# sdace9719/marl-soccer

Hardware: NVIDIA B200
Metric: env_steps_per_sec (higher is better)
Workload: dtype f32

## Files before the change

marl_soccer_b200/csrc/msoc.cu:

```cuda
#include <cuda_runtime.h>
#include <cuda_bf16.h>
#include <stdint.h>
#include <stdio.h>
#include <stdlib.h>
#include <string.h>
#include <atomic>
#include <string>
#include <vector>

#include "../../include/msoc.h"
#include "step_core.cuh"
#include "render_core.cuh"

using namespace msoc;

#ifdef MSOC_CHECKS
__device__ unsigned int g_msoc_check_bits;
#endif

static thread_local std::string g_last_error;
static std::atomic<uint64_t> g_launches{0};

static int fail(int code, const char *what, cudaError_t ce = cudaSuccess)
{
    char buf[512];
    if (ce != cudaSuccess) snprintf(buf, sizeof buf, "%s: %s", what, cudaGetErrorString(ce));
    else snprintf(buf, sizeof buf, "%s", what);
    g_last_error = buf;
    return code;
}
#define CUDA_TRY(expr)                                                        \
    do {                                                                      \
        cudaError_t _e = (expr);                                              \
        if (_e != cudaSuccess) return fail(MSOC_ERR_CUDA, #expr, _e);         \
    } while (0)

struct DeviceGuard {
    int prev = -1;
    explicit DeviceGuard(int dev) { cudaGetDevice(&prev); if (prev != dev) cudaSetDevice(dev); else prev = -1; }
    ~DeviceGuard() { if (prev >= 0) cudaSetDevice(prev); }
};

constexpr int MAX_CHUNKS = 8;
enum { CTL_LIGHT = 0, CTL_HEAVY = 1, CTL_NEXT_BATCH = 2, CTL_PAIR = 4, CTL_MULTI = 5, CTL_WORDS = 8 };
enum { CTL_STEP_FAST = 16, CTL_STEP_CONTACT = 17, CTL_LAST_COUNTS = 20 , CTL_CHUNK0 = 24, CTL_TOTAL = CTL_CHUNK0 + CTL_WORDS * MAX_CHUNKS };

struct msoc_handle {
    int device;
    int64_t n;
    uint64_t global_offset;
    SimCfg cfg;
    Arrays A;
    int sm_count, blocks_per_sm;
    int blocks_per_sm_teams;
    int heavy_lanes_override;
    void *slab;
    float *d_obs, *d_act, *d_rew;
    uint8_t *d_done, *d_mask;
    int8_t *d_goal;
    int32_t *d_score;
    double *d_stats;
    int *d_ctl;
    int *d_list;
    int *d_list2;
    float *d_frames;
    void *d_inject;
    cudaStream_t pipe_stream;
    cudaEvent_t ev_pipe_fork, ev_pipe_join;
    void *d_stage; size_t stage_bytes;
};

constexpr int WARPS_PER_BLOCK = 4;
constexpr int BLOCK = WARPS_PER_BLOCK * 32;

constexpr int ENV_STRIDE = SCRATCH_WORDS | 1;
constexpr int OBS_ENVS = 8;
constexpr int BLOCK_WORDS = OBS_ENVS * 4 * OBS;
constexpr int REC_F4 = 7;
constexpr int RECS_WORDS = OBS_ENVS * 3 * REC_F4 * 4;
constexpr int STAGE_WORDS = BLOCK_WORDS + RECS_WORDS;

struct StepParams {
    Arrays A;
    SimCfg cfg;
    const float *actions;
    float *obs_out;
    float *frames_out;
    float *reward;
    uint8_t *done;
    int8_t *goal;
    int32_t *score;
    double *stats;
    int *ctl;
    int *list;
    int *list2;
    int64_t e0, e1;
    uint64_t global_offset;
    uint32_t flags;
    int heavy_lanes;
    int chunk;
};

#ifdef MSOC_TIMELINE
__device__ unsigned long long g_tl[1 << 18];
__device__ unsigned int g_tl_n;
extern "C" int msoc_debug_timeline(unsigned long long *out, unsigned int *n) {
    cudaMemcpyFromSymbol(n, g_tl_n, sizeof(unsigned int)); unsigned int z = 0; cudaMemcpyToSymbol(g_tl_n, &z, sizeof z);
    return (int)cudaMemcpyFromSymbol(out, g_tl, sizeof g_tl);
}
__device__ __forceinline__ unsigned long long gtime() { unsigned long long t; asm volatile("mov.u64 %0, %%globaltimer;" : "=l"(t)); return t; }
__device__ __forceinline__ void tl_record(int kid, unsigned long long t0) {
    const unsigned int i = atomicAdd(&g_tl_n, 1u);
    unsigned int smid; asm volatile("mov.u32 %0, %%smid;" : "=r"(smid));
    if (i < (1u << 16)) { g_tl[4 * i] = (unsigned long long)kid; g_tl[4 * i + 1] = t0; g_tl[4 * i + 2] = gtime(); g_tl[4 * i + 3] = smid; }
}
#define MSOC_TL_BEGIN() const unsigned long long tl0 = gtime()
#define MSOC_TL_END(kid) do { if (lane == 0) tl_record(kid, tl0); } while (0)
#else
#define MSOC_TL_BEGIN() do { } while (0)
#define MSOC_TL_END(kid) do { } while (0)
#endif
struct Tally { int done, goals_b, goals_r, contacts, overflow, nonfinite; float ret; };
__device__ __forceinline__ void tally_clear(Tally &T) { T.done = T.goals_b = T.goals_r = T.contacts = T.overflow = T.nonfinite = 0; T.ret = 0.0f; }

__device__ __forceinline__ int *step_ctl(const StepParams &P, int step) { return P.chunk < 0 ? P.ctl + CTL_WORDS * (step & 1) : P.ctl + CTL_CHUNK0 + CTL_WORDS * P.chunk; }

template <bool TEAMS>
__device__ __forceinline__ bool step_one_env(const int MODE, const int ALLOWED, const StepParams &P, int step, int64_t e, Work &W, int &load, Tally &T)
{
    float act[12];
    const float4 *a4 = reinterpret_cast<const float4 *>(P.actions + e * 12);
    const float4 x0 = __ldg(a4), x1 = __ldg(a4 + 1), x2 = __ldg(a4 + 2);
    act[0] = x0.x; act[1] = x0.y; act[2] = x0.z; act[3] = x0.w;
    act[4] = x1.x; act[5] = x1.y; act[6] = x1.z; act[7] = x1.w;
    act[8] = x2.x; act[9] = x2.y; act[10] = x2.z; act[11] = x2.w;
    bool finite = true;
#pragma unroll
    for (int k = 0; k < 12; k++) finite = finite && (fabsf(act[k]) <= 3.0e38f);
    Env E;
    const float4 *rec = P.A.pose[buf_cur(step)] + e * POSE_F4;
    if ((ALLOWED & (1 << MODE_FULL)) && MODE == MODE_FULL) {
        if (__float_as_uint(rec[7].z) & FLAG_INJECT) rec = P.A.inject + e * POSE_F4;
    }
    load_env(P.A, rec, e, E);
    StepOut out;
    if (!env_step<TEAMS>(MODE, ALLOWED, E, act, P.cfg, P.A, cache_half(step), e, P.global_offset + (uint64_t)e, P.flags, W, out, load)) return false;
    if (TEAMS) reinterpret_cast<float4 *>(P.reward)[e] = make_float4(out.reward, out.reward, out.reward_r, out.reward_r);
    else reinterpret_cast<float2 *>(P.reward)[e] = make_float2(out.reward, out.reward);
    P.done[e] = out.done;
    P.goal[e] = out.goal;
    if (P.score != nullptr) reinterpret_cast<int2 *>(P.score)[e] = make_int2(out.score_b, out.score_r);
    store_env(P.A, buf_next(step), e, E, out.score_dirty);
    if (out.fresh_episode) {
        store_env_record(P.A.pose[buf_cur(step)] + e * POSE_F4, E);
        store_env_record(P.A.pose[buf_prev(step)] + e * POSE_F4, E);
    }
    T.nonfinite += finite ? 0 : 1;
    T.done += out.done; T.goals_b += out.goal > 0; T.goals_r += out.goal < 0;
    T.contacts += out.n_contacts; T.overflow += out.overflow; T.ret += out.finished_return;
    return true;
}

__device__ __forceinline__ void bulk_store(void *gdst, const void *ssrc, uint32_t bytes)
{
    asm volatile("cp.async.bulk.global.shared::cta.bulk_group [%0], [%1], %2;" ::"l"(gdst), "r"((uint32_t)__cvta_generic_to_shared(ssrc)), "r"(bytes) : "memory");
}
__device__ __forceinline__ void bulk_commit() { asm volatile("cp.async.bulk.commit_group;" ::: "memory"); }
__device__ __forceinline__ void bulk_wait_read() { asm volatile("cp.async.bulk.wait_group.read 0;" ::: "memory"); }
__device__ __forceinline__ void fence_async_smem() { asm volatile("fence.proxy.async.shared::cta;" ::: "memory"); }

struct RecLoad { float4 v[6]; };
__device__ __forceinline__ void fetch_slot(int r, int lane, int &k, int &e8, int &f)
{
    const int sl = r * 32 + lane;
    k = sl / (OBS_ENVS * REC_F4);
    const int rem = sl - k * (OBS_ENVS * REC_F4);
    e8 = rem / REC_F4; f = rem - e8 * REC_F4;
}
__device__ __forceinline__ void obs_fetch(const Arrays &A, int step, uint32_t mask, int g, int my_env, int lane, RecLoad &R)
{
    const uint32_t m8 = (mask >> (8 * g)) & 0xffu;
#pragma unroll
    for (int r = 0; r < 6; r++) {
        int k, e8, f;
        fetch_slot(r, lane, k, e8, f);
        const int env = __shfl_sync(0xffffffffu, my_env, (8 * g + e8) & 31);
        R.v[r] = make_float4(0.0f, 0.0f, 0.0f, 0.0f);
        if ((r < 5 || lane < 3 * OBS_ENVS * REC_F4 - 160) && ((m8 >> e8) & 1u)) {
            const int b = k == 0 ? buf_prev(step) : k == 1 ? buf_cur(step) : buf_next(step);
            const float4 *p = A.pose[b] + (int64_t)env * POSE_F4 + f;
            R.v[r] = k == 2 ? __ldcg(p) : *p;
        }
    }
}
__device__ __forceinline__ void obs_tile(const Arrays &A, const SimCfg &cfg, float *obs_out, float *frames_out, int step, float *s_stage,
                                         uint32_t lane_mask, int64_t my_env64, int lane)
{
    const int a = lane & 3, el = lane >> 2;
    float4 *recs4 = reinterpret_cast<float4 *>(s_stage + BLOCK_WORDS);
    float2 *mine = reinterpret_cast<float2 *>(s_stage) + lane * 33;
    __syncwarp();
    uint32_t mask = lane_mask;
    int my_env = (int)my_env64;
    if (lane_mask != 0xffffffffu) {
        int *s_idx = reinterpret_cast<int *>(s_stage);
        if ((lane_mask >> lane) & 1u) s_idx[__popc(lane_mask & ((1u << lane) - 1u))] = my_env;
        __syncwarp();
// ... 8 lines not shown
#pragma unroll 1
    while (true) {
        const uint32_t m8 = (mask >> (8 * g)) & 0xffu;
#pragma unroll
        for (int r = 0; r < 6; r++)
            if (r < 5 || lane < 3 * OBS_ENVS * REC_F4 - 160) recs4[r * 32 + lane] = R.v[r];
        __syncwarp();
        int gn = g + 1;
        while (gn < 4 && ((mask >> (8 * gn)) & 0xffu) == 0u) gn++;
        if (gn < 4) obs_fetch(A, step, mask, gn, my_env, lane, R);
        const int env = __shfl_sync(0xffffffffu, my_env, 8 * g + el);
        if ((m8 >> el) & 1u) {
            MSOC_CHECK(env >= 0 && env < A.n, CHK_OBS_ENV);
#pragma unroll
            for (int k = 0; k < 3; k++) {
                float o[22];
                frame_of_record(recs4 + (k * OBS_ENVS + el) * REC_F4, a, cfg, o);
#pragma unroll
                for (int i = 0; i < 11; i++) mine[k * 11 + i] = make_float2(o[2 * i], o[2 * i + 1]);
            }
        }
        fence_async_smem();
        __syncwarp();
        if (a == 0 && ((m8 >> el) & 1u))
            bulk_store(obs_out + (int64_t)env * (4 * OBS), s_stage + el * (4 * OBS), 4 * OBS * sizeof(float));
        bulk_commit();
        if (frames_out != nullptr) {
            float2 *fr2 = reinterpret_cast<float2 *>(frames_out);
            const float2 *stage2 = reinterpret_cast<const float2 *>(s_stage);
#pragma unroll
            for (int it = 0; it < 11; it++) {
                const int idx = it * 32 + lane;
                const int row = idx / 11, j = idx - row * 11;
                const int env2 = __shfl_sync(0xffffffffu, my_env, 8 * g + (row >> 2));
                if ((m8 >> (row >> 2)) & 1u) fr2[(int64_t)env2 * 44 + (row & 3) * 11 + j] = stage2[row * 33 + 22 + j];
            }
        }
        bulk_wait_read();
        __syncwarp();
        if (gn >= 4) break;
        g = gn;
    }
}

#ifndef MSOC_FAST_BLOCK
#define MSOC_FAST_BLOCK 128
#endif
constexpr int FAST_BLOCK = MSOC_FAST_BLOCK;
constexpr size_t FAST_SMEM_BYTES = (size_t)(FAST_BLOCK / 32) * STAGE_WORDS * sizeof(float);
#ifndef MSOC_FAST_MIN_BLOCKS
#define MSOC_FAST_MIN_BLOCKS 4
#endif

__device__ __forceinline__ void flush_tally(const Tally &T, double *stats, int lane)
{
    int nd = T.done, gb = T.goals_b, gr = T.goals_r, nc = T.contacts, ov = T.overflow, nf = T.nonfinite;
    float ret = T.ret;
    if (!__any_sync(0xffffffffu, (nd | gb | gr | nc | ov | nf) != 0)) return;
#pragma unroll
    for (int o = 16; o > 0; o >>= 1) {
        nd += __shfl_xor_sync(0xffffffffu, nd, o); gb += __shfl_xor_sync(0xffffffffu, gb, o);
        gr += __shfl_xor_sync(0xffffffffu, gr, o); nc += __shfl_xor_sync(0xffffffffu, nc, o);
        ov += __shfl_xor_sync(0xffffffffu, ov, o);
        nf += __shfl_xor_sync(0xffffffffu, nf, o);
        ret += __shfl_xor_sync(0xffffffffu, ret, o);
    }
    if (lane == 0) {
        if (nd) { atomicAdd(stats + 0, (double)nd); atomicAdd(stats + 1, (double)ret); }
        if (gb) atomicAdd(stats + 2, (double)gb);
        if (gr) atomicAdd(stats + 3, (double)gr);
        if (nc) atomicAdd(stats + 5, (double)nc);
        if (ov) atomicAdd(stats + 6, (double)ov);
        if (nf) atomicAdd(stats + 7, (double)nf);
    }
}

template <bool TEAMS>
__global__ void __launch_bounds__(FAST_BLOCK, MSOC_FAST_MIN_BLOCKS) msoc_step_fast_kernel(const __grid_constant__ StepParams P)
{
    extern __shared__ __align__(16) float s_dyn[];
    const int tid = threadIdx.x, warp = tid >> 5, lane = tid & 31;
    float *s_warp = s_dyn + warp * STAGE_WORDS;
    cudaGridDependencySynchronize();
    const int step = P.ctl[CTL_STEP_FAST];
    int *ctl = step_ctl(P, step);
    if (blockIdx.x == 0) {
        if (P.chunk < 0 && tid < CTL_WORDS) P.ctl[CTL_WORDS * ((step & 1) ^ 1) + tid] = 0;
        if (tid == 0) {
            P.ctl[CTL_STEP_CONTACT] = step;
            atomicAdd(P.stats + 4, (double)(P.e1 - P.e0));
        }
    }
    MSOC_TL_BEGIN();
    const int64_t my_env = P.e0 + (int64_t)blockIdx.x * FAST_BLOCK + tid;
    const bool have = my_env < P.e1;
    Tally T; tally_clear(T);
    Work W;
    W.ovf = nullptr; W.body = W.pool = W.geom = W.old = W.isl = nullptr; W.pool_count = nullptr;
    bool ok = false;
    int load = 0;
    if (have) {
        asm volatile("prefetch.global.L2 [%0];" ::"l"(P.A.pose[buf_prev(step)] + my_env * POSE_F4));
        ok = step_one_env<TEAMS>(MODE_FAST, 1 << MODE_FAST, P, step, my_env, W, load, T);
    }
    const uint32_t mask = __ballot_sync(0xffffffffu, ok);
    const bool declined = have && !ok;
    const uint32_t mdec = __ballot_sync(0xffffffffu, declined);
    uint32_t mclass = 0u;
    int base = 0;
    if (mdec != 0u) {
        const uint32_t b0 = __ballot_sync(0xffffffffu, declined && (load & 1)), b1 = __ballot_sync(0xffffffffu, declined && (load & 2));
        auto class_mask = [&](int cl) { return mdec & ((cl & 1) ? b0 : ~b0) & ((cl & 2) ? b1 : ~b1); };
        mclass = class_mask(load);
        const uint32_t of_lane = class_mask(lane & 3);
        if (lane < N_LOADS && of_lane != 0u) {
            const int word = lane == LOAD_LIGHT ? CTL_LIGHT : lane == LOAD_HEAVY ? CTL_HEAVY : lane == LOAD_PAIR ? CTL_PAIR : CTL_MULTI;
            base = atomicAdd(ctl + word, __popc(of_lane));
        }
    }
    if (mask != 0u) obs_tile(P.A, P.cfg, P.obs_out, P.frames_out, step, s_warp, mask, my_env, lane);
    if (mdec != 0u) {
        base = __shfl_sync(0xffffffffu, base, declined ? load : 0);
        if (declined) {
            const int rank = base + __popc(mclass & ((1u << lane) - 1u));
            int *lst = (load == LOAD_LIGHT || load == LOAD_HEAVY) ? P.list : P.list2;
            const bool front = load == LOAD_LIGHT || load == LOAD_PAIR;
            lst[front ? P.e0 + rank : P.e1 - 1 - rank] = (int)my_env;
        }
    }
    flush_tally(T, P.stats, lane);
    if ((blockIdx.x & 15) == 0 && warp == 0) MSOC_TL_END(0);
}

static_assert(STAGE_WORDS <= 32 * ENV_STRIDE, "the observation staging must fit the per-warp solver scratch");
#ifndef MSOC_HEAVY_BLOCK
#define MSOC_HEAVY_BLOCK 64
#endif
constexpr int HEAVY_BLOCK = MSOC_HEAVY_BLOCK;
#ifndef MSOC_HEAVY_MIN_BLOCKS
#define MSOC_HEAVY_MIN_BLOCKS 4
#endif
constexpr int HEAVY_MIN_BLOCKS = MSOC_HEAVY_MIN_BLOCKS;

constexpr int HEAVY_WARP_WORDS = (32 * ENV_STRIDE + 3) & ~3;
constexpr size_t STEP_SMEM_BYTES = (size_t)(HEAVY_BLOCK / 32) * HEAVY_WARP_WORDS * sizeof(float);

template <int MODES, bool TEAMS>
__device__ __forceinline__ void contact_body(const StepParams &P, int *s_pool_count)
{
    extern __shared__ __align__(16) float s_dyn[];
    const int tid = threadIdx.x, warp = tid >> 5, lane = tid & 31;
    float *s_warp = s_dyn + warp * HEAVY_WARP_WORDS;
    cudaGridDependencySynchronize();
    const int step = P.ctl[CTL_STEP_CONTACT];
    int *ctl = step_ctl(P, step);
    if (P.chunk < 0 && blockIdx.x == 0 && tid == 0) {
        P.ctl[CTL_STEP_FAST] = (step + 1) % 6;
        P.ctl[CTL_LAST_COUNTS + 0] = ctl[CTL_LIGHT]; P.ctl[CTL_LAST_COUNTS + 1] = ctl[CTL_HEAVY];
        P.ctl[CTL_LAST_COUNTS + 2] = ctl[CTL_PAIR]; P.ctl[CTL_LAST_COUNTS + 3] = ctl[CTL_MULTI];
    }
    const int n_heavy = (MODES & (1 << MODE_FULL)) ? ctl[CTL_HEAVY] : 0, n_multi = (MODES & (1 << MODE_MULTI)) ? ctl[CTL_MULTI] : 0;
    const int n_pair = (MODES & (1 << MODE_PAIR)) ? ctl[CTL_PAIR] : 0, n_light = (MODES & (1 << MODE_LIGHT)) ? ctl[CTL_LIGHT] : 0;
    MSOC_CHECK(step >= 0 && step < 6, CHK_STEP_COUNTER);
    MSOC_CHECK(n_heavy >= 0 && n_light >= 0 && (int64_t)n_heavy + n_light <= P.e1 - P.e0, CHK_LIST_COUNT);
    MSOC_CHECK(n_multi >= 0 && n_pair >= 0 && (int64_t)n_multi + n_pair <= P.e1 - P.e0, CHK_LIST_COUNT);
    int heavy_lanes = P.heavy_lanes;
    if (heavy_lanes == 0) {
        const int n_warps_ = gridDim.x * (HEAVY_BLOCK / 32);
        heavy_lanes = 1;
        while (heavy_lanes < 32 && heavy_lanes * n_warps_ < n_heavy) heavy_lanes *= 2;
        if (heavy_lanes >= 8) heavy_lanes = heavy_lanes >= 16 ? 32 : 16;
    }
    const int b_heavy = (n_heavy + heavy_lanes - 1) / heavy_lanes;
    const int b_multi = b_heavy + (n_multi + 31) / 32, b_pair = b_multi + (n_pair + 31) / 32;
    const int batches = b_pair + (n_light + 31) / 32;

    Tally T; tally_clear(T);
    float ovf_store[MAXC - CON_FAST][CON_FIELDS];
    Work W;
    W.ovf = ovf_store;
    W.body = s_warp + lane;
    W.pool = s_warp + BODY_FIELDS * 5 * 32;
    W.pool_count = s_pool_count + warp;
    W.geom = s_warp + (BODY_FIELDS * 5 + CON_FIELDS * CON_FAST) * 32 + lane;
    W.old = s_warp + (BODY_FIELDS * 5 + CON_FIELDS * CON_FAST + GEOM_WORDS) * 32 + lane;
    W.isl = s_warp + BODY_FIELDS * 5 * 32 + lane;
    const int n_warps = gridDim.x * (HEAVY_BLOCK / 32);
    int b = blockIdx.x * (HEAVY_BLOCK / 32) + warp;
#pragma unroll 1
    while (b < batches) {
        int mode, idx, count, lanes = 32;
        const int *slot;
        if (b < b_heavy)      { mode = MODE_FULL;  lanes = heavy_lanes; idx = b * lanes + lane;  count = n_heavy; slot = P.list + (P.e1 - 1 - idx); }
        else if (b < b_multi) { mode = MODE_MULTI; idx = (b - b_heavy) * 32 + lane; count = n_multi; slot = P.list2 + (P.e1 - 1 - idx); }
        else if (b < b_pair)  { mode = MODE_PAIR;  idx = (b - b_multi) * 32 + lane; count = n_pair;  slot = P.list2 + (P.e0 + idx); }
        else                  { mode = MODE_LIGHT; idx = (b - b_pair) * 32 + lane;  count = n_light; slot = P.list + (P.e0 + idx); }
        const bool have = lane < lanes && idx < count;
        const int64_t my_env = have ? (int64_t)*slot : 0;
        MSOC_CHECK(!have || (my_env >= P.e0 && my_env < P.e1), CHK_LIST_ENV);
        MSOC_TL_BEGIN();
        bool ok = false;
        int load = 0;
        if (lane == 0) *W.pool_count = 0;
        __syncwarp();
        if (have) {
            asm volatile("prefetch.global.L2 [%0];" ::"l"(P.A.pose[buf_prev(step)] + my_env * POSE_F4));
            ok = step_one_env<TEAMS>(mode, MODES, P, step, my_env, W, load, T);
        }
        const uint32_t mask = __ballot_sync(0xffffffffu, ok);
        if (mask != 0u) obs_tile(P.A, P.cfg, P.obs_out, P.frames_out, step, s_warp, mask, my_env, lane);
        MSOC_TL_END(mode == MODE_FULL ? 2 : mode == MODE_LIGHT ? 1 : 3);
        if (lane == 0) b = n_warps + atomicAdd(ctl + CTL_NEXT_BATCH, 1);
        b = __shfl_sync(0xffffffffu, b, 0);
    }
    flush_tally(T, P.stats, lane);
}

template <bool TEAMS>
__global__ void __launch_bounds__(HEAVY_BLOCK, HEAVY_MIN_BLOCKS) msoc_step_contact_kernel(const __grid_constant__ StepParams P)
{
    __shared__ int s_pool_count[HEAVY_BLOCK / 32];
    contact_body<(1 << MODE_FULL) | (1 << MODE_LIGHT) | (1 << MODE_PAIR) | (1 << MODE_MULTI), TEAMS>(P, s_pool_count);
}

__global__ void msoc_advance_kernel(int *ctl)
{
    if (threadIdx.x == 0) ctl[CTL_STEP_FAST] = (ctl[CTL_STEP_FAST] + 1) % 6;
    if (threadIdx.x < 4) {
        const int word = threadIdx.x == 0 ? CTL_LIGHT : threadIdx.x == 1 ? CTL_HEAVY : threadIdx.x == 2 ? CTL_PAIR : CTL_MULTI;
        int sum = 0;
        for (int c = 0; c < MAX_CHUNKS; c++) sum += ctl[CTL_CHUNK0 + CTL_WORDS * c + word];
        ctl[CTL_LAST_COUNTS + threadIdx.x] = sum;
    }
}

struct ResetParams {
    Arrays A;
    SimCfg cfg;
    const uint8_t *mask;
    float *obs_out;
    const int *ctl;
    uint64_t global_offset, seed;
    int mode, has_seed;
};

__global__ void __launch_bounds__(BLOCK) msoc_reset_kernel(const __grid_constant__ ResetParams P)
{
    __shared__ __align__(16) float s_stage[WARPS_PER_BLOCK][STAGE_WORDS];
    const int warp = threadIdx.x >> 5, lane = threadIdx.x & 31;
    const int64_t block_base = (int64_t)blockIdx.x * BLOCK;
    const int64_t e = block_base + threadIdx.x;
    if (block_base + warp * 32 >= P.A.n) return;
    const int step = P.ctl[CTL_STEP_FAST];
    const bool doit = (e < P.A.n) && (P.mask == nullptr || P.mask[e] != 0);
    if (doit) {
        const uint64_t gidx = P.global_offset + (uint64_t)e;
        uint64_t seed; uint32_t sc;
        if (P.has_seed) { seed = P.seed + gidx; sc = 0; P.A.seed[e] = seed; }
        else { seed = P.A.seed[e]; sc = P.A.spawn_count[e]; }
        Env E;
        env_full_reset(E, P.mode, seed, gidx, sc);
        P.A.spawn_count[e] = sc;
        store_env(P.A, buf_cur(step), e, E, true);
        store_env_record(P.A.pose[buf_prev(step)] + e * POSE_F4, E);
        store_env_record(P.A.pose[buf_next(step)] + e * POSE_F4, E);
    }
    const uint32_t m = __ballot_sync(0xffffffffu, doit);
    if (P.obs_out != nullptr && m != 0u) obs_tile(P.A, P.cfg, P.obs_out, nullptr, step, s_stage[warp], m, e, lane);
}

enum { CHK_STATES = CHK_RENDER + 1 };
constexpr int STATE_ENVS = 8;
constexpr int STATE_WORDS = (int)(sizeof(msoc_env_state) / 4);
constexpr int STATE_GROUP_U4 = STATE_ENVS * STATE_WORDS / 4;
constexpr int STATE_BLOCK = 128;
static_assert(sizeof(msoc_env_state) == 808 && (STATE_ENVS * sizeof(msoc_env_state)) % 16 == 0, "msoc_env_state layout");
enum : int {
    SW_POS = offsetof(msoc_env_state, pos) / 4, SW_VEL = offsetof(msoc_env_state, vel) / 4,
    SW_ANG = offsetof(msoc_env_state, ang) / 4, SW_ANGVEL = offsetof(msoc_env_state, angvel) / 4,
    SW_VBIAS = offsetof(msoc_env_state, vbias) / 4, SW_RET = offsetof(msoc_env_state, ep_return) / 4,
    SW_STEPS = offsetof(msoc_env_state, steps) / 4, SW_SCORE = offsetof(msoc_env_state, score) / 4,
    SW_MODE = offsetof(msoc_env_state, mode) / 4, SW_SPAWN = offsetof(msoc_env_state, spawn_count) / 4,
    SW_CCOUNT = offsetof(msoc_env_state, cache_count) / 4, SW_SEED = offsetof(msoc_env_state, seed) / 4,
    SW_CINFO = offsetof(msoc_env_state, cache_info) / 4, SW_HVALID = offsetof(msoc_env_state, hist_valid) / 4,
    SW_HPOS = offsetof(msoc_env_state, hist_pos) / 4, SW_HVEL = offsetof(msoc_env_state, hist_vel) / 4,
    SW_HANG = offsetof(msoc_env_state, hist_ang) / 4, SW_HANGVEL = offsetof(msoc_env_state, hist_angvel) / 4,
};
static_assert(offsetof(msoc_env_state, wbias) == offsetof(msoc_env_state, vbias) + 40 && offsetof(msoc_env_state, cache_jn) == offsetof(msoc_env_state, cache_info) + 128,
              "msoc_env_state layout");

struct StateParams {
    Arrays A;
    const int *ctl;
    const int64_t *idx;
    int64_t n;
    uint8_t *states;
};

__device__ __forceinline__ void group_store(uint8_t *g, const uint32_t *s, int count, int lane)
{
    const int valid = count * (int)sizeof(msoc_env_state);
    const uint4 *s4 = reinterpret_cast<const uint4 *>(s);
#pragma unroll
    for (int i = 0; i < (STATE_GROUP_U4 + 31) / 32; i++) {
        const int k = i * 32 + lane, off = k * 16;
        if (off + 16 <= valid) reinterpret_cast<uint4 *>(g)[k] = s4[k];
        else if (off < valid) reinterpret_cast<uint2 *>(g + off)[0] = reinterpret_cast<const uint2 *>(s4 + k)[0];
    }
}
__device__ __forceinline__ void group_load(uint32_t *s, const uint8_t *g, int count, int lane)
{
    const int valid = count * (int)sizeof(msoc_env_state);
    uint4 *s4 = reinterpret_cast<uint4 *>(s);
#pragma unroll
    for (int i = 0; i < (STATE_GROUP_U4 + 31) / 32; i++) {
        const int k = i * 32 + lane, off = k * 16;
        if (off + 16 <= valid) s4[k] = __ldcs(reinterpret_cast<const uint4 *>(g) + k);
        else if (off < valid) reinterpret_cast<uint2 *>(s4 + k)[0] = __ldcs(reinterpret_cast<const uint2 *>(g + off));
    }
}

__device__ __forceinline__ void put_state_f4(uint32_t *w, int f, float4 v)
{
    if (f < 5) {
        w[SW_POS + 2 * f] = __float_as_uint(v.x); w[SW_POS + 2 * f + 1] = __float_as_uint(v.y);
        w[SW_VEL + 2 * f] = __float_as_uint(v.z); w[SW_VEL + 2 * f + 1] = __float_as_uint(v.w);
    } else if (f < 7) {
        const int o = f == 5 ? SW_ANG : SW_ANGVEL;
        w[o] = __float_as_uint(v.x); w[o + 1] = __float_as_uint(v.y); w[o + 2] = __float_as_uint(v.z); w[o + 3] = __float_as_uint(v.w);
    } else {
        const uint32_t flags = __float_as_uint(v.z);
        w[SW_ANGVEL + 4] = __float_as_uint(v.x); w[SW_STEPS] = __float_as_uint(v.y); w[SW_RET] = __float_as_uint(v.w);
        w[SW_MODE] = (flags & FLAG_MODE_MASK) >> FLAG_MODE_SHIFT; w[SW_CCOUNT] = flags & FLAG_CACHE_MASK;
    }
}
__device__ __forceinline__ void put_hist_f4(uint32_t *w, int k, int f, float4 v)
{
    if (f < 5) {
        w[SW_HPOS + 10 * k + 2 * f] = __float_as_uint(v.x); w[SW_HPOS + 10 * k + 2 * f + 1] = __float_as_uint(v.y);
        if (f < 4) { w[SW_HVEL + 8 * k + 2 * f] = __float_as_uint(v.z); w[SW_HVEL + 8 * k + 2 * f + 1] = __float_as_uint(v.w); }
    } else {
        const int o = (f == 5 ? SW_HANG : SW_HANGVEL) + 4 * k;
        w[o] = __float_as_uint(v.x); w[o + 1] = __float_as_uint(v.y); w[o + 2] = __float_as_uint(v.z); w[o + 3] = __float_as_uint(v.w);
    }
}
__device__ __forceinline__ float state_angle(uint32_t bits)
{
    const float a = __uint_as_float(bits);
    return (a > PI_F || a < -PI_F) ? wrap_angle(a) : a;
}
__device__ __forceinline__ float4 get_state_f4(const uint32_t *w, int f, uint32_t flags)
{
    if (f < 5) return make_float4(__uint_as_float(w[SW_POS + 2 * f]), __uint_as_float(w[SW_POS + 2 * f + 1]),
                                  __uint_as_float(w[SW_VEL + 2 * f]), __uint_as_float(w[SW_VEL + 2 * f + 1]));
    if (f == 5) return make_float4(state_angle(w[SW_ANG]), state_angle(w[SW_ANG + 1]), state_angle(w[SW_ANG + 2]), state_angle(w[SW_ANG + 3]));
    if (f == 6) return make_float4(__uint_as_float(w[SW_ANGVEL]), __uint_as_float(w[SW_ANGVEL + 1]), __uint_as_float(w[SW_ANGVEL + 2]), __uint_as_float(w[SW_ANGVEL + 3]));
    return make_float4(__uint_as_float(w[SW_ANGVEL + 4]), __uint_as_float(w[SW_STEPS]), __uint_as_float(flags), __uint_as_float(w[SW_RET]));
}
__device__ __forceinline__ float4 get_hist_f4(const uint32_t *w, int k, int f)
{
    if (f < 4) return make_float4(__uint_as_float(w[SW_HPOS + 10 * k + 2 * f]), __uint_as_float(w[SW_HPOS + 10 * k + 2 * f + 1]),
                                  __uint_as_float(w[SW_HVEL + 8 * k + 2 * f]), __uint_as_float(w[SW_HVEL + 8 * k + 2 * f + 1]));
    if (f == 4) return make_float4(__uint_as_float(w[SW_HPOS + 10 * k + 8]), __uint_as_float(w[SW_HPOS + 10 * k + 9]), 0.0f, 0.0f);
    const int o = SW_HANG + 4 * k;
    if (f == 5) return make_float4(state_angle(w[o]), state_angle(w[o + 1]), state_angle(w[o + 2]), state_angle(w[o + 3]));
    const int p = SW_HANGVEL + 4 * k;
    return make_float4(__uint_as_float(w[p]), __uint_as_float(w[p + 1]), __uint_as_float(w[p + 2]), __uint_as_float(w[p + 3]));
}
__device__ __forceinline__ bool same_pose_f4(int f, float4 a, float4 b)
{
    bool same = __float_as_uint(a.x) == __float_as_uint(b.x) && __float_as_uint(a.y) == __float_as_uint(b.y);
    if (f != 4) same = same && __float_as_uint(a.z) == __float_as_uint(b.z) && __float_as_uint(a.w) == __float_as_uint(b.w);
    return same;
}
__device__ __forceinline__ int64_t state_env(const StateParams &P, int64_t t, bool &ok)
// ... 237 lines not shown
                const int row = rem / P.G.W, col = rem - row * P.G.W;
                const int count = g_end - g0 < RENDER_SEG ? (int)(g_end - g0) : RENDER_SEG;
                uint32_t wm, bm, rm, ym, zm;
                render_segment_masks(P.G, s_scene, img, row, col, count, wm, bm, rm, ym, zm);
                render_pack(wm, bm, rm, ym, zm, w);
                uint4 *st4 = reinterpret_cast<uint4 *>(stage + lane * RENDER_SEG_WORDS);
#pragma unroll
                for (int i = 0; i < RENDER_SEG_WORDS / 4; i++) st4[i] = make_uint4(w[4 * i], w[4 * i + 1], w[4 * i + 2], w[4 * i + 3]);
            }
            __syncwarp();
            const int64_t byte0 = warp_g0 * 3;
            const int64_t valid = (g_end - warp_g0) * 3 < 32 * RENDER_SEG * 3 ? (g_end - warp_g0) * 3 : 32 * RENDER_SEG * 3;
            const uint4 *src = reinterpret_cast<const uint4 *>(stage);
#pragma unroll
            for (int i = 0; i < RENDER_SEG_WORDS / 4; i++) {
                const int off = (i * 32 + lane) * 16;
                if (off + 16 <= valid) {
                    MSOC_CHECK(byte0 + off + 16 <= P.total_px * 3, CHK_RENDER);
                    __stcs(reinterpret_cast<uint4 *>(P.out + byte0 + off), src[i * 32 + lane]);
                } else if (off < valid) {
                    const uint8_t *sb = reinterpret_cast<const uint8_t *>(src + i * 32 + lane);
                    for (int b = 0; b < valid - off; b++) P.out[byte0 + off + b] = sb[b];
                }
            }
            __syncwarp();
        }
    }
}

template <int TEAM>
static int launch_policy_inputs(const float *d_obs, int64_t n_envs, const float *d_shift, const float *d_inv_std, void *d_x_out,
                                void *d_raw_out, double *d_moments, void *stream)
{
    int dev = 0, sms = 0;
    CUDA_TRY(cudaGetDevice(&dev));
    CUDA_TRY(cudaDeviceGetAttribute(&sms, cudaDevAttrMultiProcessorCount, dev));
    const int64_t want = (n_envs + PI_Y - 1) / PI_Y, cap = (int64_t)sms * 7;
    msoc_policy_inputs_kernel<TEAM><<<(unsigned)(want < cap ? want : cap), dim3(PI_X, PI_Y), 0, (cudaStream_t)stream>>>(
        d_obs, n_envs, d_shift, d_inv_std, (__nv_bfloat162 *)d_x_out, (__nv_bfloat162 *)d_raw_out, d_moments);
    g_launches++;
    CUDA_TRY(cudaGetLastError());
    return MSOC_OK;
}

extern "C" {

const char *msoc_last_error(void) { return g_last_error.c_str(); }
int msoc_version(void) { return MSOC_VERSION; }
uint64_t msoc_launch_count(void) { return g_launches.load(); }
int msoc_debug_errors(void)
{
#ifdef MSOC_CHECKS
    unsigned int bits = 0, zero = 0;
    if (cudaDeviceSynchronize() != cudaSuccess) return -2;
    if (cudaMemcpyFromSymbol(&bits, g_msoc_check_bits, sizeof bits) != cudaSuccess) return -2;
    cudaMemcpyToSymbol(g_msoc_check_bits, &zero, sizeof zero);
    return (int)bits;
#else
    return -1;
#endif
}
int64_t msoc_num_envs(const msoc_handle *h) { return h ? h->n : 0; }

static size_t align_up(size_t x) { return (x + 255) & ~(size_t)255; }

static int grid_for(int64_t n) { return (int)((n + BLOCK - 1) / BLOCK); }

static void fill_cfg(const msoc_config *c, SimCfg &s)
{
    s.max_velocity = c->max_velocity;
    s.agent_minv = 1.0f / c->agent_mass; s.ball_minv = 1.0f / c->ball_mass;
    s.agent_iinv = 1.0f / c->agent_moment; s.ball_iinv = 1.0f / c->ball_moment;
    s.agent_friction = c->agent_friction; s.ball_friction = c->ball_friction;
    s.force_max = c->action_force_max; s.torque_max = c->action_torque_max;
    s.max_ang_vel = c->max_angular_velocity;
    s.prox_mult = c->ball_proximity_multiplier; s.move_mult = c->move_ball_to_goal_multiplier;
    s.goal_reward = c->goal_scored_reward; s.conceded_penalty = c->goal_conceded_penalty;
    s.alive_penalty = c->alive_penalty; s.score_diff_mult = c->score_difference_multiplier;
    s.max_steps = c->max_steps; s.pad = 0;
    cfg_derive(s);
}

int msoc_reset(msoc_handle *h, const uint8_t *d_mask, int mode, int has_seed, uint64_t seed, float *d_obs_out, void *stream);
int msoc_destroy(msoc_handle *h);

int msoc_create(const msoc_config *cfg, int64_t n_envs, int device, uint64_t seed, uint64_t global_env_offset,
                msoc_handle **out)
{
    if (!cfg || !out || n_envs <= 0) return fail(MSOC_ERR_INVALID, "msoc_create: bad argument");
    if (n_envs > 0x7fffffff) return fail(MSOC_ERR_INVALID, "msoc_create: at most 2^31 - 1 envs per handle");
    if (!(cfg->agent_mass > 0.0f) || !(cfg->ball_mass > 0.0f) || !(cfg->agent_moment > 0.0f) || !(cfg->ball_moment > 0.0f))
        return fail(MSOC_ERR_INVALID, "msoc_create: masses and moments must be positive");
    int ndev = 0;
    cudaError_t ce = cudaGetDeviceCount(&ndev);
    if (ce != cudaSuccess || ndev <= 0)
        return fail(MSOC_ERR_CUDA, "msoc_create: no CUDA device (this library has no CPU fallback)", ce);
    if (device < 0 || device >= ndev) return fail(MSOC_ERR_INVALID, "msoc_create: bad device index");
    DeviceGuard guard(device);

    msoc_handle *h = new msoc_handle();
    memset(h, 0, sizeof *h);
    h->device = device; h->n = n_envs; h->global_offset = global_env_offset;
    fill_cfg(cfg, h->cfg);
    if (const char *hl = getenv("MSOC_HEAVY_LANES")) {
        const int v = atoi(hl);
        if (v == 1 || v == 2 || v == 4 || v == 8 || v == 16 || v == 32) h->heavy_lanes_override = v;
    }
    auto bail = [&](int code, const char *what, cudaError_t e) { msoc_destroy(h); return fail(code, what, e); };

    const size_t n = (size_t)n_envs;
    size_t off = 0;
    auto take = [&](size_t bytes) { size_t o = off; off += align_up(bytes); return o; };
    size_t o_pose[3], o_cache[2];
    for (int k = 0; k < 3; k++) o_pose[k] = take(n * POSE_F4 * sizeof(float4));
    const size_t o_iscore = take(n * sizeof(int2));
    const size_t o_bias = take(n * 4 * sizeof(float4));
    const size_t o_seed = take(n * sizeof(uint64_t)), o_sc = take(n * sizeof(uint32_t));
    for (int k = 0; k < 2; k++) o_cache[k] = take(n * MAX_CACHE * 3 * sizeof(uint32_t));
    const size_t o_obs = take(n * 4 * OBS * sizeof(float)), o_act = take(n * 12 * sizeof(float));
    const size_t o_rew = take(n * 2 * sizeof(float)), o_done = take(n), o_goal = take(n), o_mask = take(n);
    const size_t o_score = take(n * 2 * sizeof(int32_t));
    const size_t o_stats = take(8 * sizeof(double));
    const size_t o_ctl = take(CTL_TOTAL * sizeof(int));
    const size_t o_list = take(n * sizeof(int)), o_list2 = take(n * sizeof(int));
    const size_t total = off;

    ce = cudaMalloc(&h->slab, total);
    if (ce != cudaSuccess) return bail(MSOC_ERR_ALLOC, "msoc_create: cudaMalloc", ce);
    ce = cudaMemset(h->slab, 0, total);
    if (ce != cudaSuccess) return bail(MSOC_ERR_CUDA, "msoc_create: cudaMemset", ce);
    char *base = (char *)h->slab;
    Arrays &A = h->A;
    A.n = n_envs;
    for (int k = 0; k < 3; k++) A.pose[k] = (float4 *)(base + o_pose[k]);
    for (int k = 0; k < 2; k++) A.cache[k] = (uint32_t *)(base + o_cache[k]);
    A.score = (int2 *)(base + o_iscore);
    A.bias = (float4 *)(base + o_bias);
    A.inject = nullptr;
    A.seed = (uint64_t *)(base + o_seed); A.spawn_count = (uint32_t *)(base + o_sc);
    h->d_obs = (float *)(base + o_obs); h->d_act = (float *)(base + o_act); h->d_rew = (float *)(base + o_rew);
    h->d_done = (uint8_t *)(base + o_done); h->d_goal = (int8_t *)(base + o_goal); h->d_mask = (uint8_t *)(base + o_mask);
    h->d_score = (int32_t *)(base + o_score);
    h->d_stats = (double *)(base + o_stats);
    h->d_ctl = (int *)(base + o_ctl);
    h->d_list = (int *)(base + o_list); h->d_list2 = (int *)(base + o_list2);

    ce = cudaFuncSetAttribute(msoc_step_contact_kernel<false>, cudaFuncAttributeMaxDynamicSharedMemorySize, (int)STEP_SMEM_BYTES);
    if (ce == cudaSuccess)
        ce = cudaFuncSetAttribute(msoc_step_fast_kernel<false>, cudaFuncAttributeMaxDynamicSharedMemorySize, (int)FAST_SMEM_BYTES);
    if (ce == cudaSuccess)
        ce = cudaFuncSetAttribute(msoc_step_contact_kernel<true>, cudaFuncAttributeMaxDynamicSharedMemorySize, (int)STEP_SMEM_BYTES);
    if (ce == cudaSuccess)
        ce = cudaFuncSetAttribute(msoc_step_fast_kernel<true>, cudaFuncAttributeMaxDynamicSharedMemorySize, (int)FAST_SMEM_BYTES);
    if (ce != cudaSuccess) return bail(MSOC_ERR_CUDA, "msoc_create: smem attribute", ce);
    cudaDeviceGetAttribute(&h->sm_count, cudaDevAttrMultiProcessorCount, device);
    ce = cudaOccupancyMaxActiveBlocksPerMultiprocessor(&h->blocks_per_sm, msoc_step_contact_kernel<false>, HEAVY_BLOCK, STEP_SMEM_BYTES);
    if (ce == cudaSuccess)
        ce = cudaOccupancyMaxActiveBlocksPerMultiprocessor(&h->blocks_per_sm_teams, msoc_step_contact_kernel<true>, HEAVY_BLOCK, STEP_SMEM_BYTES);
    if (ce != cudaSuccess || h->blocks_per_sm < 1 || h->blocks_per_sm_teams < 1 || h->sm_count < 1)
        return bail(MSOC_ERR_CUDA, "msoc_create: occupancy query", ce);
    if (ce == cudaSuccess) ce = cudaStreamCreateWithFlags(&h->pipe_stream, cudaStreamNonBlocking);
    if (ce == cudaSuccess) ce = cudaEventCreateWithFlags(&h->ev_pipe_fork, cudaEventDisableTiming);
    if (ce == cudaSuccess) ce = cudaEventCreateWithFlags(&h->ev_pipe_join, cudaEventDisableTiming);
    if (ce != cudaSuccess) return bail(MSOC_ERR_CUDA, "msoc_create: stream/event", ce);
    msoc_init_kernel<<<(unsigned)((n_envs + 255) / 256), 256>>>(A, seed);
    g_launches++;
    int rc = msoc_reset(h, nullptr, MSOC_MODE_RANDOM, 0, 0, h->d_obs, nullptr);
    if (rc != MSOC_OK) { msoc_destroy(h); return rc; }
    ce = cudaDeviceSynchronize();
    if (ce != cudaSuccess) return bail(MSOC_ERR_CUDA, "msoc_create: init", ce);
    *out = h;
    return MSOC_OK;
}

int msoc_destroy(msoc_handle *h)
{
    if (!h) return MSOC_OK;
    DeviceGuard guard(h->device);
    cudaDeviceSynchronize();
    if (h->d_stage) cudaFree(h->d_stage);
    if (h->d_frames) cudaFree(h->d_frames);
    if (h->d_inject) cudaFree(h->d_inject);
    if (h->ev_pipe_fork) cudaEventDestroy(h->ev_pipe_fork);
    if (h->ev_pipe_join) cudaEventDestroy(h->ev_pipe_join);
    if (h->pipe_stream) cudaStreamDestroy(h->pipe_stream);
    if (h->slab) cudaFree(h->slab);
    delete h;
    return MSOC_OK;
}

int msoc_reset(msoc_handle *h, const uint8_t *d_mask, int mode, int has_seed, uint64_t seed, float *d_obs_out, void *stream)
{
    if (!h) return fail(MSOC_ERR_INVALID, "msoc_reset: null handle");
    if (mode < 0 || mode > 2) return fail(MSOC_ERR_INVALID, "msoc_reset: bad mode");
    DeviceGuard guard(h->device);
    ResetParams P;
    P.A = h->A; P.cfg = h->cfg; P.mask = d_mask; P.obs_out = d_obs_out; P.ctl = h->d_ctl;
    P.global_offset = h->global_offset; P.seed = seed; P.mode = mode; P.has_seed = has_seed;
    msoc_reset_kernel<<<grid_for(h->n), BLOCK, 0, (cudaStream_t)stream>>>(P);
    g_launches++;
    CUDA_TRY(cudaGetLastError());
    return MSOC_OK;
}

static int launch_step(msoc_handle *h, StepParams &P, int64_t e0, int64_t e1, int chunk, cudaStream_t st, bool teams = false)
{
    P.e0 = e0; P.e1 = e1; P.chunk = chunk;
    const int64_t m = e1 - e0;
    P.heavy_lanes = h->heavy_lanes_override;
    cudaLaunchAttribute at[1];
    at[0].id = cudaLaunchAttributeProgrammaticStreamSerialization;
    at[0].val.programmaticStreamSerializationAllowed = 1;
    cudaLaunchConfig_t lf = {};
    lf.gridDim = dim3((unsigned)((m + FAST_BLOCK - 1) / FAST_BLOCK));
    lf.blockDim = dim3(FAST_BLOCK);
    lf.dynamicSmemBytes = FAST_SMEM_BYTES;
    lf.stream = st;
    lf.attrs = at; lf.numAttrs = 1;
    CUDA_TRY(cudaLaunchKernelEx(&lf, teams ? msoc_step_fast_kernel<true> : msoc_step_fast_kernel<false>, P));
    g_launches++;
    const int64_t resident = (int64_t)h->sm_count * (teams ? h->blocks_per_sm_teams : h->blocks_per_sm);
    const int64_t blocks_max = (m + HEAVY_BLOCK - 1) / HEAVY_BLOCK;
    cudaLaunchConfig_t lc = {};
    lc.gridDim = dim3((unsigned)(blocks_max < resident ? blocks_max : resident));
    lc.blockDim = dim3(HEAVY_BLOCK);
    lc.dynamicSmemBytes = STEP_SMEM_BYTES;
    lc.stream = st;
    lc.attrs = at; lc.numAttrs = 1;
    CUDA_TRY(cudaLaunchKernelEx(&lc, teams ? msoc_step_contact_kernel<true> : msoc_step_contact_kernel<false>, P));
    g_launches++;
    return MSOC_OK;
}

static void fill_step_params(msoc_handle *h, StepParams &P, const float *d_actions, float *d_obs_out, float *d_frames_out,
                             float *d_reward, uint8_t *d_done, int8_t *d_goal, int32_t *d_score, uint32_t flags)
{
    P.A = h->A; P.cfg = h->cfg; P.actions = d_actions; P.obs_out = d_obs_out; P.frames_out = d_frames_out;
    P.reward = d_reward; P.done = d_done; P.goal = d_goal; P.score = d_score; P.stats = h->d_stats;
    P.global_offset = h->global_offset; P.flags = flags;
    P.ctl = h->d_ctl; P.list = h->d_list; P.list2 = h->d_list2;
}

int msoc_step(msoc_handle *h, const float *d_actions, float *d_obs_out, float *d_reward,
              uint8_t *d_done, int8_t *d_goal, int32_t *d_score, uint32_t flags, void *stream)
{
    if (!h || !d_actions || !d_obs_out || !d_reward || !d_done || !d_goal)
        return fail(MSOC_ERR_INVALID, "msoc_step: null argument");
    DeviceGuard guard(h->device);
    StepParams P;
    fill_step_params(h, P, d_actions, d_obs_out, nullptr, d_reward, d_done, d_goal, d_score, flags);
    return launch_step(h, P, 0, h->n, -1, (cudaStream_t)stream);
}

int msoc_step_teams(msoc_handle *h, const float *d_actions, float *d_obs_out, float *d_reward,
                    uint8_t *d_done, int8_t *d_goal, int32_t *d_score, uint32_t flags, void *stream)
{
    if (!h || !d_actions || !d_obs_out || !d_reward || !d_done || !d_goal)
        return fail(MSOC_ERR_INVALID, "msoc_step_teams: null argument");
    if ((uintptr_t)d_reward & 15u) return fail(MSOC_ERR_INVALID, "msoc_step_teams: d_reward must be 16-byte aligned");
    DeviceGuard guard(h->device);
    StepParams P;
    fill_step_params(h, P, d_actions, d_obs_out, nullptr, d_reward, d_done, d_goal, d_score, flags);
    return launch_step(h, P, 0, h->n, -1, (cudaStream_t)stream, true);
}

static int step_host_impl(msoc_handle *h, const float *h_actions, float *h_obs, float *h_frames, float *h_reward, uint8_t *h_done,
                          int8_t *h_goal, int32_t *h_score, uint32_t flags, void *stream)
{
    if (!h || !h_actions) return fail(MSOC_ERR_INVALID, "msoc_step_host: null argument");
    DeviceGuard guard(h->device);
    cudaStream_t st = (cudaStream_t)stream;
    if (h_frames && !h->d_frames) {
        cudaError_t ce = cudaMalloc(&h->d_frames, (size_t)h->n * 4 * FRAME * sizeof(float));
        if (ce != cudaSuccess) return fail(MSOC_ERR_ALLOC, "msoc_step_host_frames: cudaMalloc", ce);
    }
    StepParams P;
    fill_step_params(h, P, h->d_act, h->d_obs, h_frames ? h->d_frames : nullptr, h->d_rew, h->d_done, h->d_goal, h->d_score, flags);
    int chunks = (int)(h->n / 65536);
    if (chunks < 1) chunks = 1;
    if (chunks > MAX_CHUNKS) chunks = MAX_CHUNKS;
    const int64_t per = ((h->n + chunks - 1) / chunks + 127) & ~(int64_t)127;
    auto copies_back = [&](int64_t e0, int64_t m, cudaStream_t s) -> int {
        if (h_obs) CUDA_TRY(cudaMemcpyAsync(h_obs + e0 * 4 * OBS, h->d_obs + e0 * 4 * OBS, (size_t)m * 4 * OBS * sizeof(float), cudaMemcpyDeviceToHost, s));
        if (h_frames) CUDA_TRY(cudaMemcpyAsync(h_frames + e0 * 4 * FRAME, h->d_frames + e0 * 4 * FRAME, (size_t)m * 4 * FRAME * sizeof(float), cudaMemcpyDeviceToHost, s));
        if (h_reward) CUDA_TRY(cudaMemcpyAsync(h_reward + e0 * 2, h->d_rew + e0 * 2, (size_t)m * 2 * sizeof(float), cudaMemcpyDeviceToHost, s));
        if (h_done) CUDA_TRY(cudaMemcpyAsync(h_done + e0, h->d_done + e0, (size_t)m, cudaMemcpyDeviceToHost, s));
        if (h_goal) CUDA_TRY(cudaMemcpyAsync(h_goal + e0, h->d_goal + e0, (size_t)m, cudaMemcpyDeviceToHost, s));
        if (h_score) CUDA_TRY(cudaMemcpyAsync(h_score + e0 * 2, h->d_score + e0 * 2, (size_t)m * 2 * sizeof(int32_t), cudaMemcpyDeviceToHost, s));
        return MSOC_OK;
    };
    if (chunks == 1) {
        CUDA_TRY(cudaMemcpyAsync(h->d_act, h_actions, (size_t)h->n * 12 * sizeof(float), cudaMemcpyHostToDevice, st));
        int rc = launch_step(h, P, 0, h->n, -1, st);
        if (rc != MSOC_OK) return rc;
        rc = copies_back(0, h->n, st);
        if (rc != MSOC_OK) return rc;
        CUDA_TRY(cudaStreamSynchronize(st));
        return MSOC_OK;
    }
    CUDA_TRY(cudaMemsetAsync(h->d_ctl + CTL_CHUNK0, 0, CTL_WORDS * MAX_CHUNKS * sizeof(int), st));
    CUDA_TRY(cudaEventRecord(h->ev_pipe_fork, st));
    CUDA_TRY(cudaStreamWaitEvent(h->pipe_stream, h->ev_pipe_fork, 0));
    for (int c = 0; c < chunks; c++) {
        const int64_t e0 = c * per, e1 = (e0 + per < h->n) ? e0 + per : h->n;
        if (e0 >= e1) break;
        cudaStream_t s = (c & 1) ? h->pipe_stream : st;
        CUDA_TRY(cudaMemcpyAsync(h->d_act + e0 * 12, h_actions + e0 * 12, (size_t)(e1 - e0) * 12 * sizeof(float), cudaMemcpyHostToDevice, s));
        int rc = launch_step(h, P, e0, e1, c, s);
        if (rc != MSOC_OK) return rc;
        rc = copies_back(e0, e1 - e0, s);
        if (rc != MSOC_OK) return rc;
    }
    CUDA_TRY(cudaEventRecord(h->ev_pipe_join, h->pipe_stream));
    CUDA_TRY(cudaStreamWaitEvent(st, h->ev_pipe_join, 0));
    msoc_advance_kernel<<<1, 32, 0, st>>>(h->d_ctl);
    g_launches++;
    CUDA_TRY(cudaGetLastError());
    CUDA_TRY(cudaStreamSynchronize(st));
    return MSOC_OK;
}

int msoc_step_host(msoc_handle *h, const float *h_actions, float *h_obs, float *h_reward, uint8_t *h_done,
                   int8_t *h_goal, int32_t *h_score, uint32_t flags, void *stream)
{
    return step_host_impl(h, h_actions, h_obs, nullptr, h_reward, h_done, h_goal, h_score, flags, stream);
}

int msoc_step_host_frames(msoc_handle *h, const float *h_actions, float *h_frames, float *h_reward, uint8_t *h_done,
                          int8_t *h_goal, int32_t *h_score, uint32_t flags, void *stream)
{
    if (!h_frames) return fail(MSOC_ERR_INVALID, "msoc_step_host_frames: null frame buffer");
    return step_host_impl(h, h_actions, nullptr, h_frames, h_reward, h_done, h_goal, h_score, flags, stream);
}

int msoc_reset_host(msoc_handle *h, const uint8_t *h_mask, int mode, int has_seed, uint64_t seed, float *h_obs, void *stream)
{
    if (!h) return fail(MSOC_ERR_INVALID, "msoc_reset_host: null handle");
    DeviceGuard guard(h->device);
    cudaStream_t st = (cudaStream_t)stream;
    const size_t n = (size_t)h->n;
    if (h_mask) CUDA_TRY(cudaMemcpyAsync(h->d_mask, h_mask, n, cudaMemcpyHostToDevice, st));
    int rc = msoc_reset(h, h_mask ? h->d_mask : nullptr, mode, has_seed, seed, h->d_obs, stream);
    if (rc != MSOC_OK) return rc;
    if (h_obs) CUDA_TRY(cudaMemcpyAsync(h_obs, h->d_obs, n * 4 * OBS * sizeof(float), cudaMemcpyDeviceToHost, st));
    CUDA_TRY(cudaStreamSynchronize(st));
    return MSOC_OK;
}

int msoc_read_counters(msoc_handle *h, int32_t *h_score, int32_t *h_steps, void *stream)
{
    if (!h) return fail(MSOC_ERR_INVALID, "msoc_read_counters: null handle");
    DeviceGuard guard(h->device);
    cudaStream_t st = (cudaStream_t)stream;
    int step = 0;
    CUDA_TRY(cudaMemcpyAsync(&step, h->d_ctl + CTL_STEP_FAST, sizeof(int), cudaMemcpyDeviceToHost, st));
    CUDA_TRY(cudaStreamSynchronize(st));
    if (h_steps) {
        std::vector<float4> tmp((size_t)h->n);
        CUDA_TRY(cudaMemcpy2DAsync(tmp.data(), sizeof(float4), h->A.pose[step % 3] + 7, POSE_F4 * sizeof(float4), sizeof(float4), (size_t)h->n, cudaMemcpyDeviceToHost, st));
        CUDA_TRY(cudaStreamSynchronize(st));
        for (int64_t i = 0; i < h->n; i++) { int32_t v; memcpy(&v, &tmp[(size_t)i].y, 4); h_steps[i] = v; }
    }
    if (h_score) {
        CUDA_TRY(cudaMemcpyAsync(h_score, h->A.score, (size_t)h->n * sizeof(int2), cudaMemcpyDeviceToHost, st));
        CUDA_TRY(cudaStreamSynchronize(st));
    }
    return MSOC_OK;
}

static int ensure_stage(msoc_handle *h, size_t bytes)
{
    if (h->stage_bytes >= bytes) return MSOC_OK;
    if (h->d_stage) cudaFree(h->d_stage);
    h->d_stage = nullptr; h->stage_bytes = 0;
    cudaError_t ce = cudaMalloc(&h->d_stage, bytes);
    if (ce != cudaSuccess) return fail(MSOC_ERR_ALLOC, "state staging cudaMalloc", ce);
    h->stage_bytes = bytes;
    return MSOC_OK;
}

static int check_idx(const msoc_handle *h, const int64_t *idx, int64_t n, const char *who)
{
    if (!h || !idx || n <= 0) return fail(MSOC_ERR_INVALID, who);
// ... 249 lines not shown
```

Measured before the change: 2.070 billion.

## Split light-mode envs into a separate low-smem kernel overlapped via PDL

Moves MODE_LIGHT environments out of the heavy contact kernel into a new light kernel. The new kernel uses a small staging buffer and no contact work buffers, so it can run at higher occupancy. The contact kernel now triggers programmatic launch completion early, so the light kernel can start while it is still running; the light kernel defers its grid dependency sync to the end. This adds a launch and a separate batch counter (CTL_NEXT_LIGHT). It risks ordering hazards if the counters are not reset or the two kernels share state, and it sets a max-shared carveout.

```diff
diff --git a/marl_soccer_b200/csrc/msoc.cu b/marl_soccer_b200/csrc/msoc.cu
--- a/marl_soccer_b200/csrc/msoc.cu
+++ b/marl_soccer_b200/csrc/msoc.cu
@@ -42,7 +42,7 @@
 };
 
 constexpr int MAX_CHUNKS = 8;
-enum { CTL_LIGHT = 0, CTL_HEAVY = 1, CTL_NEXT_BATCH = 2, CTL_PAIR = 4, CTL_MULTI = 5, CTL_WORDS = 8 };
+enum { CTL_LIGHT = 0, CTL_HEAVY = 1, CTL_NEXT_BATCH = 2, CTL_NEXT_LIGHT = 3, CTL_PAIR = 4, CTL_MULTI = 5, CTL_WORDS = 8 };
 enum { CTL_STEP_FAST = 16, CTL_STEP_CONTACT = 17, CTL_LAST_COUNTS = 20 , CTL_CHUNK0 = 24, CTL_TOTAL = CTL_CHUNK0 + CTL_WORDS * MAX_CHUNKS };
 
 struct msoc_handle {
@@ -53,6 +53,7 @@
     Arrays A;
     int sm_count, blocks_per_sm;
     int blocks_per_sm_teams;
+    int light_blocks_per_sm, light_blocks_per_sm_teams;
     int heavy_lanes_override;
     void *slab;
     float *d_obs, *d_act, *d_rew;
@@ -367,6 +368,7 @@
     const int tid = threadIdx.x, warp = tid >> 5, lane = tid & 31;
     float *s_warp = s_dyn + warp * HEAVY_WARP_WORDS;
     cudaGridDependencySynchronize();
+    cudaTriggerProgrammaticLaunchCompletion();
     const int step = P.ctl[CTL_STEP_CONTACT];
     int *ctl = step_ctl(P, step);
     if (P.chunk < 0 && blockIdx.x == 0 && tid == 0) {
@@ -375,9 +377,9 @@
         P.ctl[CTL_LAST_COUNTS + 2] = ctl[CTL_PAIR]; P.ctl[CTL_LAST_COUNTS + 3] = ctl[CTL_MULTI];
     }
     const int n_heavy = (MODES & (1 << MODE_FULL)) ? ctl[CTL_HEAVY] : 0, n_multi = (MODES & (1 << MODE_MULTI)) ? ctl[CTL_MULTI] : 0;
-    const int n_pair = (MODES & (1 << MODE_PAIR)) ? ctl[CTL_PAIR] : 0, n_light = (MODES & (1 << MODE_LIGHT)) ? ctl[CTL_LIGHT] : 0;
+    const int n_pair = (MODES & (1 << MODE_PAIR)) ? ctl[CTL_PAIR] : 0;
     MSOC_CHECK(step >= 0 && step < 6, CHK_STEP_COUNTER);
-    MSOC_CHECK(n_heavy >= 0 && n_light >= 0 && (int64_t)n_heavy + n_light <= P.e1 - P.e0, CHK_LIST_COUNT);
+    MSOC_CHECK(n_heavy >= 0 && ctl[CTL_LIGHT] >= 0 && (int64_t)n_heavy + ctl[CTL_LIGHT] <= P.e1 - P.e0, CHK_LIST_COUNT);
     MSOC_CHECK(n_multi >= 0 && n_pair >= 0 && (int64_t)n_multi + n_pair <= P.e1 - P.e0, CHK_LIST_COUNT);
     int heavy_lanes = P.heavy_lanes;
     if (heavy_lanes == 0) {
@@ -387,8 +389,7 @@
         if (heavy_lanes >= 8) heavy_lanes = heavy_lanes >= 16 ? 32 : 16;
     }
     const int b_heavy = (n_heavy + heavy_lanes - 1) / heavy_lanes;
-    const int b_multi = b_heavy + (n_multi + 31) / 32, b_pair = b_multi + (n_pair + 31) / 32;
-    const int batches = b_pair + (n_light + 31) / 32;
+    const int b_multi = b_heavy + (n_multi + 31) / 32, batches = b_multi + (n_pair + 31) / 32;
 
     Tally T; tally_clear(T);
     float ovf_store[MAXC - CON_FAST][CON_FIELDS];
@@ -408,8 +409,7 @@
         const int *slot;
         if (b < b_heavy)      { mode = MODE_FULL;  lanes = heavy_lanes; idx = b * lanes + lane;  count = n_heavy; slot = P.list + (P.e1 - 1 - idx); }
         else if (b < b_multi) { mode = MODE_MULTI; idx = (b - b_heavy) * 32 + lane; count = n_multi; slot = P.list2 + (P.e1 - 1 - idx); }
-        else if (b < b_pair)  { mode = MODE_PAIR;  idx = (b - b_multi) * 32 + lane; count = n_pair;  slot = P.list2 + (P.e0 + idx); }
-        else                  { mode = MODE_LIGHT; idx = (b - b_pair) * 32 + lane;  count = n_light; slot = P.list + (P.e0 + idx); }
+        else                  { mode = MODE_PAIR;  idx = (b - b_multi) * 32 + lane; count = n_pair;  slot = P.list2 + (P.e0 + idx); }
         const bool have = lane < lanes && idx < count;
         const int64_t my_env = have ? (int64_t)*slot : 0;
         MSOC_CHECK(!have || (my_env >= P.e0 && my_env < P.e1), CHK_LIST_ENV);
@@ -424,7 +424,7 @@
         }
         const uint32_t mask = __ballot_sync(0xffffffffu, ok);
         if (mask != 0u) obs_tile(P.A, P.cfg, P.obs_out, P.frames_out, step, s_warp, mask, my_env, lane);
-        MSOC_TL_END(mode == MODE_FULL ? 2 : mode == MODE_LIGHT ? 1 : 3);
+        MSOC_TL_END(mode == MODE_FULL ? 2 : 3);
         if (lane == 0) b = n_warps + atomicAdd(ctl + CTL_NEXT_BATCH, 1);
         b = __shfl_sync(0xffffffffu, b, 0);
     }
@@ -435,7 +435,53 @@
 __global__ void __launch_bounds__(HEAVY_BLOCK, HEAVY_MIN_BLOCKS) msoc_step_contact_kernel(const __grid_constant__ StepParams P)
 {
     __shared__ int s_pool_count[HEAVY_BLOCK / 32];
-    contact_body<(1 << MODE_FULL) | (1 << MODE_LIGHT) | (1 << MODE_PAIR) | (1 << MODE_MULTI), TEAMS>(P, s_pool_count);
+    contact_body<(1 << MODE_FULL) | (1 << MODE_PAIR) | (1 << MODE_MULTI), TEAMS>(P, s_pool_count);
+}
+
+#ifndef MSOC_LIGHT_BLOCK
+#define MSOC_LIGHT_BLOCK 64
+#endif
+constexpr int LIGHT_BLOCK = MSOC_LIGHT_BLOCK;
+constexpr size_t LIGHT_SMEM_BYTES = (size_t)(LIGHT_BLOCK / 32) * STAGE_WORDS * sizeof(float);
+
+template <bool TEAMS>
+__global__ void __launch_bounds__(LIGHT_BLOCK) msoc_step_light_kernel(const __grid_constant__ StepParams P)
+{
+    extern __shared__ __align__(16) float s_dyn[];
+    const int tid = threadIdx.x, warp = tid >> 5, lane = tid & 31;
+    float *s_warp = s_dyn + warp * STAGE_WORDS;
+    const int step = __ldcg(P.ctl + CTL_STEP_CONTACT);
+    int *ctl = step_ctl(P, step);
+    const int n_light = __ldcg(ctl + CTL_LIGHT);
+    MSOC_CHECK(step >= 0 && step < 6, CHK_STEP_COUNTER);
+    MSOC_CHECK(n_light >= 0 && n_light <= P.e1 - P.e0, CHK_LIST_COUNT);
+    const int batches = (n_light + 31) / 32;
+    Tally T; tally_clear(T);
+    Work W;
+    W.ovf = nullptr; W.body = W.pool = W.geom = W.old = W.isl = nullptr; W.pool_count = nullptr;
+    const int n_warps = gridDim.x * (LIGHT_BLOCK / 32);
+    int b = blockIdx.x * (LIGHT_BLOCK / 32) + warp;
+#pragma unroll 1
+    while (b < batches) {
+        const int idx = b * 32 + lane;
+        const bool have = idx < n_light;
+        const int64_t my_env = have ? (int64_t)__ldcg(P.list + (P.e0 + idx)) : 0;
+        MSOC_CHECK(!have || (my_env >= P.e0 && my_env < P.e1), CHK_LIST_ENV);
+        MSOC_TL_BEGIN();
+        bool ok = false;
+        int load = 0;
+        if (have) {
+            asm volatile("prefetch.global.L2 [%0];" ::"l"(P.A.pose[buf_prev(step)] + my_env * POSE_F4));
+            ok = step_one_env<TEAMS>(MODE_LIGHT, 1 << MODE_LIGHT, P, step, my_env, W, load, T);
+        }
+        const uint32_t mask = __ballot_sync(0xffffffffu, ok);
+        if (mask != 0u) obs_tile(P.A, P.cfg, P.obs_out, P.frames_out, step, s_warp, mask, my_env, lane);
+        MSOC_TL_END(1);
+        if (lane == 0) b = n_warps + atomicAdd(ctl + CTL_NEXT_LIGHT, 1);
+        b = __shfl_sync(0xffffffffu, b, 0);
+    }
+    flush_tally(T, P.stats, lane);
+    cudaGridDependencySynchronize();
 }
 
 __global__ void msoc_advance_kernel(int *ctl)
@@ -979,12 +1025,23 @@
         ce = cudaFuncSetAttribute(msoc_step_contact_kernel<true>, cudaFuncAttributeMaxDynamicSharedMemorySize, (int)STEP_SMEM_BYTES);
     if (ce == cudaSuccess)
         ce = cudaFuncSetAttribute(msoc_step_fast_kernel<true>, cudaFuncAttributeMaxDynamicSharedMemorySize, (int)FAST_SMEM_BYTES);
+    if (ce == cudaSuccess)
+        ce = cudaFuncSetAttribute(msoc_step_light_kernel<false>, cudaFuncAttributeMaxDynamicSharedMemorySize, (int)LIGHT_SMEM_BYTES);
+    if (ce == cudaSuccess)
+        ce = cudaFuncSetAttribute(msoc_step_light_kernel<true>, cudaFuncAttributeMaxDynamicSharedMemorySize, (int)LIGHT_SMEM_BYTES);
+    for (const void *k : {(const void *)msoc_step_contact_kernel<false>, (const void *)msoc_step_contact_kernel<true>, (const void *)msoc_step_light_kernel<false>, (const void *)msoc_step_light_kernel<true>})
+        if (ce == cudaSuccess) ce = cudaFuncSetAttribute(k, cudaFuncAttributePreferredSharedMemoryCarveout, (int)cudaSharedmemCarveoutMaxShared);
     if (ce != cudaSuccess) return bail(MSOC_ERR_CUDA, "msoc_create: smem attribute", ce);
     cudaDeviceGetAttribute(&h->sm_count, cudaDevAttrMultiProcessorCount, device);
     ce = cudaOccupancyMaxActiveBlocksPerMultiprocessor(&h->blocks_per_sm, msoc_step_contact_kernel<false>, HEAVY_BLOCK, STEP_SMEM_BYTES);
     if (ce == cudaSuccess)
         ce = cudaOccupancyMaxActiveBlocksPerMultiprocessor(&h->blocks_per_sm_teams, msoc_step_contact_kernel<true>, HEAVY_BLOCK, STEP_SMEM_BYTES);
-    if (ce != cudaSuccess || h->blocks_per_sm < 1 || h->blocks_per_sm_teams < 1 || h->sm_count < 1)
+    if (ce == cudaSuccess)
+        ce = cudaOccupancyMaxActiveBlocksPerMultiprocessor(&h->light_blocks_per_sm, msoc_step_light_kernel<false>, LIGHT_BLOCK, LIGHT_SMEM_BYTES);
+    if (ce == cudaSuccess)
+        ce = cudaOccupancyMaxActiveBlocksPerMultiprocessor(&h->light_blocks_per_sm_teams, msoc_step_light_kernel<true>, LIGHT_BLOCK, LIGHT_SMEM_BYTES);
+    if (ce != cudaSuccess || h->blocks_per_sm < 1 || h->blocks_per_sm_teams < 1 || h->light_blocks_per_sm < 1 ||
+        h->light_blocks_per_sm_teams < 1 || h->sm_count < 1)
         return bail(MSOC_ERR_CUDA, "msoc_create: occupancy query", ce);
     if (ce == cudaSuccess) ce = cudaStreamCreateWithFlags(&h->pipe_stream, cudaStreamNonBlocking);
     if (ce == cudaSuccess) ce = cudaEventCreateWithFlags(&h->ev_pipe_fork, cudaEventDisableTiming);
@@ -1056,6 +1113,16 @@
     lc.attrs = at; lc.numAttrs = 1;
     CUDA_TRY(cudaLaunchKernelEx(&lc, teams ? msoc_step_contact_kernel<true> : msoc_step_contact_kernel<false>, P));
     g_launches++;
+    const int64_t light_resident = (int64_t)h->sm_count * (teams ? h->light_blocks_per_sm_teams : h->light_blocks_per_sm);
+    const int64_t light_max = (m + LIGHT_BLOCK - 1) / LIGHT_BLOCK;
+    cudaLaunchConfig_t ll = {};
+    ll.gridDim = dim3((unsigned)(light_max < light_resident ? light_max : light_resident));
+    ll.blockDim = dim3(LIGHT_BLOCK);
+    ll.dynamicSmemBytes = LIGHT_SMEM_BYTES;
+    ll.stream = st;
+    ll.attrs = at; ll.numAttrs = 1;
+    CUDA_TRY(cudaLaunchKernelEx(&ll, teams ? msoc_step_light_kernel<true> : msoc_step_light_kernel<false>, P));
+    g_launches++;
     return MSOC_OK;
 }
 
```

Result: slower. 1.931 billion, median of 6 (-6.7%).
